# 2646207530/hamer-yolo

Measured on AMD Instinct MI355X. Metric: hands/sec (HaMeR ViT-H/16 + decoder + MANO forward; detector bypassed), higher is better.
Workload: dtype fp16; 1 GPU; BASELINE configs[1]: batch=64 synthetic 256x256 crops per GPU, HaMeR ViT-H/16 + 6-layer decoder + MANO, 16-bit MFMA (fp16 operands), crops resident in HBM; batch_per_gpu=64, global_batch=64, batches_in_flight=2, weights=seeded random-init fp32 master weights, rounded to the operand type at load, parallelism=crop-shard x1

## Files before the change

hamer_yolo_amd/csrc/attention.hip:

```cpp
#include "common.h"
#include "hamer_hip_internal.h"

namespace {

constexpr int T = 192;
constexpr int HD = 80;
constexpr int KSTR = 88;
constexpr int VSTR = 80;
constexpr int KS_BYTES = T * KSTR * 2;
constexpr int VT_BYTES = T * VSTR * 2;
constexpr int BUF_BYTES = KS_BYTES + VT_BYTES;
constexpr int NWAVE = T / 16;
constexpr int OTILE_BYTES = 16 * HD * 2;
constexpr int ATT_LDS = 2 * BUF_BYTES + NWAVE * OTILE_BYTES;
constexpr int ATT_LDS_TOME = ATT_LDS + 2 * T * 4;

template <class V4> __device__ __forceinline__ V4 lds_read_tr4(const void* p) {
  typedef __attribute__((ext_vector_type(4))) short s16x4;
  const s16x4 v = __builtin_amdgcn_ds_read_tr16_b64_v4i16((__attribute__((address_space(3))) s16x4*)p);
  return __builtin_bit_cast(V4, v);
}

__device__ __forceinline__ void glds16_hidden(const void* gsrc, void* lds_wave_base) {
  const unsigned dst = __builtin_amdgcn_readfirstlane((unsigned)(uintptr_t)(__attribute__((address_space(3))) void*)lds_wave_base);
  asm volatile("s_mov_b32 m0, %1\n\ts_nop 0\n\tglobal_load_lds_dwordx4 %0, off" :: "v"(gsrc), "s"(dst) : "memory");
}

__device__ __forceinline__ void wait_vm0() {
  __builtin_amdgcn_s_waitcnt(0x0F70);
  asm volatile("" ::: "memory");
}

constexpr int HDP = 96;
typedef __attribute__((ext_vector_type(4))) int v4i_att;

template <class TT, bool MX8 = false, bool TOME = false>
__global__ __launch_bounds__(64 * NWAVE, 3) void vit_attention_kernel(const typename TT::elem* __restrict__ qkv,
                                                                    typename TT::elem* __restrict__ out, int heads,
                                                                    int items, float scale_log2e,
                                                                    unsigned char* __restrict__ out_scales = nullptr,
                                                                    const float* __restrict__ size = nullptr, int Tn = T) {
  extern __shared__ __attribute__((aligned(16))) char smem[];
  using elem = typename TT::elem;
  using vec8 = typename TT::vec8;
  using vec4 = typename TT::vec4;

  const int tid = threadIdx.x, lane = tid & 63;
  const int wave = __builtin_amdgcn_readfirstlane(tid >> 6);
  const int C = heads * HD;
  const size_t ld = (size_t)3 * C;
  const int g = lane >> 4, li = lane & 15;
  const int Tt = TOME ? Tn : T;
  vec8 zero8;
#pragma unroll
  for (int i = 0; i < 8; ++i) zero8[i] = (elem)0.0f;
  if constexpr (TOME) {
    for (int buf = 0; buf < 2; ++buf) {
      char* Vb = smem + buf * BUF_BYTES + KS_BYTES;
      for (int c = Tt * (VSTR / 8) + tid; c < T * (VSTR / 8); c += 64 * NWAVE) *(vec8*)(Vb + c * 16) = zero8;
    }
  }

  auto issue = [&](int item, int buf, vec8 (&qf)[3], float& szl) {
    const elem* base = qkv + (size_t)(item / heads) * Tt * ld + (size_t)(item % heads) * HD;
    char* Kb = smem + buf * BUF_BYTES;
    char* Vb = Kb + KS_BYTES;
    constexpr int KCH = T * (KSTR / 8), VCH = T * (VSTR / 8);
    const int kch = Tt * (KSTR / 8), vch = Tt * (VSTR / 8);
    for (int c0 = wave * 64; c0 < KCH; c0 += 64 * NWAVE) {
      const int c = c0 + lane, ch = c % (KSTR / 8);
      int t = c / (KSTR / 8);
      if (TOME) t = t < Tt ? t : Tt - 1;
      if (!TOME || c0 < kch) glds16_hidden(base + (size_t)t * ld + C + (ch < HD / 8 ? ch : 0) * 8, Kb + c0 * 16);
    }
    for (int c0 = wave * 64; c0 < VCH; c0 += 64 * NWAVE) {
      const int c = c0 + lane, ch = c % (VSTR / 8);
      int t = c / (VSTR / 8);
      if (TOME) t = t < Tt ? t : Tt - 1;
      if (!TOME || c0 < vch) glds16_hidden(base + (size_t)t * ld + 2 * C + ch * 8, Vb + c0 * 16);
    }
    const int qr = wave * 16 + li;
    const elem* qrow = base + (size_t)(TOME ? (qr < Tt ? qr : Tt - 1) : qr) * ld;
    if constexpr (TOME) szl = (size != nullptr && tid < Tt) ? size[(size_t)(item / heads) * Tt + tid] : 1.0f;
    qf[0] = *(const vec8*)(qrow + 8 * g);
    qf[1] = *(const vec8*)(qrow + 32 + 8 * g);
    qf[2] = g < 2 ? *(const vec8*)(qrow + 64 + 8 * g) : zero8;
  };

  auto compute = [&](int item, int buf, const vec8 (&qf)[3]) {
    const elem* Ks = (const elem*)(smem + buf * BUF_BYTES);
    const elem* Vs = (const elem*)(smem + buf * BUF_BYTES + KS_BYTES);
    const int b = item / heads, h = item % heads;
    const int q = wave * 16 + li;
    if constexpr (TOME) { if (wave * 16 >= Tt) return; }
    f32x4_t st[12];
    vec8 kf[2][2][3];
    auto load_k = [&](int kb, int pair) {
#pragma unroll
      for (int j = 0; j < 2; ++j) {
        const elem* krow = Ks + ((pair * 2 + j) * 16 + li) * KSTR + 8 * g;
        kf[kb][j][0] = *(const vec8*)(krow);
        kf[kb][j][1] = *(const vec8*)(krow + 32);
        kf[kb][j][2] = g < 2 ? *(const vec8*)(krow + 64) : zero8;
      }
    };
    load_k(0, 0);
#pragma unroll
    for (int pair = 0; pair < 6; ++pair) {
      if (pair + 1 < 6) load_k((pair + 1) & 1, pair + 1);
#pragma unroll
      for (int j = 0; j < 2; ++j) {
        f32x4_t acc = f32x4_t{0.f, 0.f, 0.f, 0.f};
        acc = TT::mfma(kf[pair & 1][j][0], qf[0], acc);
        acc = TT::mfma(kf[pair & 1][j][1], qf[1], acc);
        acc = TT::mfma(kf[pair & 1][j][2], qf[2], acc);
        st[pair * 2 + j] = acc;
      }
    }
    if constexpr (TOME) {
#pragma unroll
      for (int kt = 0; kt < 12; ++kt) {
        const f32x4_t lz = *(const f32x4_t*)(smem + ATT_LDS + (buf * T + kt * 16 + 4 * g) * 4);
#pragma unroll
        for (int r = 0; r < 4; ++r) st[kt][r] = (kt * 16 + 4 * g + r < Tt) ? fmaf(st[kt][r], scale_log2e, lz[r]) : -INFINITY;
      }
    }
    float m = st[0][0];
#pragma unroll
    for (int kt = 0; kt < 12; ++kt)
#pragma unroll
      for (int r = 0; r < 4; ++r) m = fmaxf(m, st[kt][r]);
    m = fmaxf(m, __shfl_xor(m, 16, 64));
    m = fmaxf(m, __shfl_xor(m, 32, 64));
    const float mneg = TOME ? -m : -m * scale_log2e;
    float sum4[4] = {0.f, 0.f, 0.f, 0.f};
#pragma unroll
    for (int kt = 0; kt < 12; ++kt)
#pragma unroll
      for (int r = 0; r < 4; ++r) {
        const float p = __builtin_amdgcn_exp2f(TOME ? st[kt][r] + (mneg + 14.0f) : fmaf(st[kt][r], scale_log2e, mneg));
        st[kt][r] = p;
        sum4[r] += p;
      }
    float sum = (sum4[0] + sum4[1]) + (sum4[2] + sum4[3]);
    sum += __shfl_xor(sum, 16, 64);
    sum += __shfl_xor(sum, 32, 64);
    const float inv = 1.0f / sum;

    vec8 pf[6], pl[TOME ? 6 : 1];
#pragma unroll
    for (int kk = 0; kk < 6; ++kk)
#pragma unroll
      for (int r = 0; r < 4; ++r) {
        pf[kk][r] = (elem)st[2 * kk][r];
        pf[kk][4 + r] = (elem)st[2 * kk + 1][r];
        if constexpr (TOME) {
          pl[kk][r] = (elem)(st[2 * kk][r] - (float)pf[kk][r]);
          pl[kk][4 + r] = (elem)(st[2 * kk + 1][r] - (float)pf[kk][4 + r]);
        }
      }

    const elem* vblk = Vs + (4 * g + (li >> 2)) * VSTR + 4 * (li & 3);
    vec4 vlo[2][5], vhi[2][5];
    auto load_v = [&](int vb, int kk) {
#pragma unroll
      for (int dt = 0; dt < 5; ++dt) {
        vlo[vb][dt] = lds_read_tr4<vec4>(vblk + (32 * kk) * VSTR + dt * 16);
        vhi[vb][dt] = lds_read_tr4<vec4>(vblk + (32 * kk + 16) * VSTR + dt * 16);
      }
    };
    f32x4_t oacc[5];
#pragma unroll
    for (int dt = 0; dt < 5; ++dt) oacc[dt] = f32x4_t{0.f, 0.f, 0.f, 0.f};
    if constexpr (!TOME) load_v(0, 0);
#pragma unroll
    for (int kk = 0; kk < 6; ++kk) {
      if constexpr (TOME) load_v(kk & 1, kk);
      else if (kk + 1 < 6) load_v((kk + 1) & 1, kk + 1);
#pragma unroll
      for (int dt = 0; dt < 5; ++dt) {
        vec8 vf;
#pragma unroll
        for (int i = 0; i < 4; ++i) { vf[i] = vlo[kk & 1][dt][i]; vf[4 + i] = vhi[kk & 1][dt][i]; }
        oacc[dt] = TT::mfma(vf, pf[kk], oacc[dt]);
        if constexpr (TOME) oacc[dt] = TT::mfma(vf, pl[kk], oacc[dt]);
      }
    }
    if constexpr (MX8) {
      const int Mrows = (items / heads) * T;
      float am[3] = {0.f, 0.f, 0.f};
#pragma unroll
      for (int dt = 0; dt < 5; ++dt)
#pragma unroll
        for (int r = 0; r < 4; ++r) am[dt >> 1] = fmaxf(am[dt >> 1], fabsf(oacc[dt][r] * inv));
      unsigned sb[3];
      float isc[3];
#pragma unroll
      for (int bk = 0; bk < 3; ++bk) {
        float a = am[bk];
        a = fmaxf(a, __shfl_xor(a, 16, 64));
        a = fmaxf(a, __shfl_xor(a, 32, 64));
        sb[bk] = mx8_scale_byte(a);
        isc[bk] = mx8_inv_scale(sb[bk]);
      }
      char* ot8 = smem + 2 * BUF_BYTES + wave * OTILE_BYTES;
#pragma unroll
      for (int dt = 0; dt < 6; ++dt) {
        int p = 0;
        if (dt < 5) {
          const float sc = inv * isc[dt >> 1];
          p = mx8_pack4(oacc[dt][0] * sc, oacc[dt][1] * sc, oacc[dt][2] * sc, oacc[dt][3] * sc);
        }
        *(int*)(ot8 + li * HDP + dt * 16 + 4 * g) = p;
      }
      char* obase8 = (char*)out + ((size_t)b * T + wave * 16) * (heads * HDP) + h * HDP;
#pragma unroll
      for (int c0 = 0; c0 < 16 * (HDP / 16); c0 += 64) {
        const int c = c0 + lane;
        if (c < 16 * (HDP / 16)) {
          const int row = c / (HDP / 16), ch = c % (HDP / 16);
          *(v4i_att*)(obase8 + (size_t)row * (heads * HDP) + ch * 16) = *(const v4i_att*)(ot8 + row * HDP + ch * 16);
        }
      }
      if (g == 0) {
#pragma unroll
        for (int bk = 0; bk < 3; ++bk) out_scales[(size_t)(h * 3 + bk) * Mrows + (size_t)b * T + q] = (unsigned char)sb[bk];
      }
      return;
    }
    elem* ot = (elem*)(smem + 2 * BUF_BYTES + wave * OTILE_BYTES);
#pragma unroll
    for (int dt = 0; dt < 5; ++dt) {
      vec4 o;
#pragma unroll
      for (int r = 0; r < 4; ++r) o[r] = (elem)(oacc[dt][r] * inv);
      *(vec4*)(ot + li * HD + dt * 16 + 4 * g) = o;
    }
    elem* obase = out + ((size_t)b * Tt + wave * 16) * C + h * HD;
#pragma unroll
    for (int c0 = 0; c0 < 16 * (HD / 8); c0 += 64) {
      const int c = c0 + lane;
      if (c < 16 * (HD / 8)) {
        const int row = c / (HD / 8), ch = c % (HD / 8);
        if (!TOME || wave * 16 + row < Tt) *(vec8*)(obase + (size_t)row * C + ch * 8) = *(const vec8*)(ot + row * HD + ch * 8);
      }
    }
  };

  vec8 qa[3], qb[3];
  float sza = 1.0f, szb = 1.0f;
  auto publish_size = [&](int buf, float szl) {
    if constexpr (TOME) { if (tid < Tt) *(float*)(smem + ATT_LDS + (buf * T + tid) * 4) = __builtin_amdgcn_logf(szl); }
  };
  int item = xcd_remap(blockIdx.x, gridDim.x);
  if (item < items) issue(item, 0, qa, sza);
  while (item < items) {
    wait_vm0();
    publish_size(0, sza);
    __builtin_amdgcn_s_barrier();
    int nxt = item + gridDim.x;
    if (nxt < items) issue(nxt, 1, qb, szb);
    compute(item, 0, qa);
    item = nxt;
    if (item >= items) break;
    wait_vm0();
    publish_size(1, szb);
    __builtin_amdgcn_s_barrier();
    nxt = item + gridDim.x;
    if (nxt < items) issue(nxt, 0, qa, sza);
    compute(item, 1, qb);
    item = nxt;
  }
}

int att_grid_for(int items, int n_cu) {
  if (const int v = hm_option(HM_OPT_ATT_GRID)) n_cu = v;
  const int per = (items + n_cu - 1) / n_cu;
  return (items + per - 1) / per;
}

template <class TT, bool MX8 = false, bool TOME = false>
int launch_att(const void* qkv, void* out, int B, int heads, float scale, hipStream_t s, void* out_scales = nullptr,
               const float* size = nullptr, int Tn = T) {
  static HmLdsOnce lds_once;
  auto kern = vit_attention_kernel<TT, MX8, TOME>;
  constexpr int LDS = TOME ? ATT_LDS_TOME : ATT_LDS;
  if (const int rc = lds_once.ensure((const void*)kern, LDS, "hm_vit_attention: cannot raise dynamic LDS limit")) return rc;
  const int n_cu = hm_device_cu_count();
  if (n_cu <= 0) return hm_set_error(HM_ERR_HIP, "hm_vit_attention: cannot query the device");
  const int items = B * heads;
  const int grid = att_grid_for(items, n_cu);
  hipLaunchKernelGGL(kern, dim3(grid), dim3(64 * NWAVE), LDS, s, (const typename TT::elem*)qkv,
                     (typename TT::elem*)out, heads, items, scale * 1.44269504088896340736f, (unsigned char*)out_scales, size, Tn);
  return hm_check_launch("hm_vit_attention");
}

}

extern "C" int hm_attention_grid(int items, int cus) {
  if (items <= 0) return 0;
  return att_grid_for(items, cus > 0 ? cus : 256);
}

int hm_attention_tome_launch(const void* qkv, const float* size, void* out, int B, int tokens, int heads, float scale, int dtype,
                             hipStream_t s) {
  if (tokens < 1 || tokens > T) return hm_set_error(HM_ERR_ARG, "hm_tome_attention: 0 < tokens <= 192");
  if (dtype == HM_DTYPE_BF16) return launch_att<TBf16, false, true>(qkv, out, B, heads, scale, s, nullptr, size, tokens);
  if (dtype == HM_DTYPE_F16) return launch_att<TF16, false, true>(qkv, out, B, heads, scale, s, nullptr, size, tokens);
  return hm_set_error(HM_ERR_ARG, "hm_tome_attention: bad dtype");
}

extern "C" int hm_vit_attention(const void* qkv, void* out, int B, int tokens, int heads, int head_dim, float scale,
                                int dtype, void* stream_) {
  hipStream_t s = (hipStream_t)stream_;
  if (!qkv || !out || B <= 0 || heads <= 0) return hm_set_error(HM_ERR_ARG, "hm_vit_attention: bad arguments");
  if (tokens != T || head_dim != HD)
    return hm_set_error(HM_ERR_ARG, "hm_vit_attention: built for 192 tokens and head_dim 80 (ViT-H/16 on 256x192)");
  if (((uintptr_t)qkv | (uintptr_t)out) & 15) return hm_set_error(HM_ERR_ARG, "hm_vit_attention: 16-byte alignment");
  HmProfScope prof(HM_K_ATTENTION, 0, B, heads, head_dim, s);
  if (dtype == HM_DTYPE_BF16) return launch_att<TBf16>(qkv, out, B, heads, scale, s);
  if (dtype == HM_DTYPE_F16) return launch_att<TF16>(qkv, out, B, heads, scale, s);
  return hm_set_error(HM_ERR_ARG, "hm_vit_attention: bad dtype");
}

extern "C" int hm_vit_attention_mx8(const void* qkv, void* out8, void* out_scales, int B, int tokens, int heads, int head_dim,
                                    float scale, void* stream_) {
  hipStream_t s = (hipStream_t)stream_;
  if (!qkv || !out8 || !out_scales || B <= 0 || heads <= 0) return hm_set_error(HM_ERR_ARG, "hm_vit_attention_mx8: bad arguments");
  if (tokens != T || head_dim != HD)
    return hm_set_error(HM_ERR_ARG, "hm_vit_attention_mx8: built for 192 tokens and head_dim 80 (ViT-H/16 on 256x192)");
  if (((uintptr_t)qkv | (uintptr_t)out8 | (uintptr_t)out_scales) & 15) return hm_set_error(HM_ERR_ARG, "hm_vit_attention_mx8: 16-byte alignment");
  HmProfScope prof(HM_K_ATTENTION, 1, B, heads, head_dim, s);
  return launch_att<TBf16, true>(qkv, out8, B, heads, scale, s, out_scales);
}
```

hamer_yolo_amd/csrc/status.hip:

```cpp
#include <stdio.h>
#include <string.h>
#include "common.h"
#include "hamer_hip_internal.h"

static thread_local char g_err[512] = "";

int hm_set_error(int code, const char* msg) {
  snprintf(g_err, sizeof(g_err), "%s", msg ? msg : "");
  return code;
}

int hm_check_launch(const char* what) {
  hipError_t e = hipGetLastError();
  if (e == hipSuccess) return HM_OK;
  snprintf(g_err, sizeof(g_err), "%s: %s", what, hipGetErrorString(e));
  return HM_ERR_HIP;
}

int hm_device_cu_count(void) {
  static std::mutex mu;
  static int cus[64] = {0};
  int dev = 0;
  if (hipGetDevice(&dev) != hipSuccess) return -1;
  std::lock_guard<std::mutex> lock(mu);
  if (dev < 64 && cus[dev] > 0) return cus[dev];
  int n = 0;
  if (hipDeviceGetAttribute(&n, hipDeviceAttributeMultiprocessorCount, dev) != hipSuccess) return -1;
  if (dev < 64) cus[dev] = n;
  return n;
}

#include <atomic>
static std::atomic<int> g_opts[HM_OPT_COUNT];
int hm_option(int key) {
  return (key >= 0 && key < HM_OPT_COUNT) ? g_opts[key].load(std::memory_order_relaxed) : 0;
}
extern "C" int hm_get_option(int key) { return hm_option(key); }
extern "C" int hm_option_count(void) { return HM_OPT_COUNT; }
extern "C" int hm_set_option(int key, int value) {
  if (key < 0 || key >= HM_OPT_COUNT) return hm_set_error(HM_ERR_ARG, "hm_set_option: unknown key");
  if (value < 0) return hm_set_error(HM_ERR_ARG, "hm_set_option: value must be >= 0");
  if ((key == HM_OPT_PX_GRID || key == HM_OPT_FP8P_GRID) && value != 0 && (value < 8 || value % 8 != 0))
    return hm_set_error(HM_ERR_ARG, "hm_set_option: a persistent grid is 0 (default) or a multiple of the 8 XCDs");
  if (key == HM_OPT_GEMM_STAGGER && value > 4)
    return hm_set_error(HM_ERR_ARG, "hm_set_option: HM_OPT_GEMM_STAGGER is 0 (default), 1 (lockstep), 2 (staggered), 3 or 4 (one kernel staggered)");
  g_opts[key].store(value, std::memory_order_relaxed);
  return HM_OK;
}

extern "C" int hm_version(void) { return HM_VERSION; }
extern "C" const char* hm_last_error_string(void) { return g_err; }
```

hamer_yolo_amd/lib.py:

```python
from __future__ import annotations

import ctypes as C
import os

HERE = os.path.dirname(os.path.abspath(__file__))
LIB_PATH = os.path.join(HERE, "libhamer_hip.so")

HM_DTYPE_BF16, HM_DTYPE_F16, HM_OUT_F32 = 0, 1, 2
HM_DTYPE_F32 = 2
HM_EPI_STORE, HM_EPI_GELU, HM_EPI_RESID_F32, HM_EPI_F32, HM_EPI_SILU = 0, 1, 2, 3, 4
HM_EPI_RESID_LN, HM_EPI_LN_STORE, HM_EPI_LN_GELU, HM_EPI_GELU_MX8 = 5, 6, 7, 8
HM_VERSION = 402
OPTION_NAMES = ("HM_OPT_PX_GRID", "HM_OPT_FP8P_GRID", "HM_OPT_FP8_ONE_TILE", "HM_OPT_FP8P_RESID", "HM_OPT_TOME_NO_SPLITK",
                "HM_OPT_TOME_SCALAR_ATTENTION", "HM_OPT_RESID_IN_EPILOGUE", "HM_OPT_CONV_TILE", "HM_OPT_CONV_SPLITK",
                "HM_OPT_PX_LDS_EPILOGUE", "HM_OPT_CONV_DIRECT", "HM_OPT_GEMM_TILE_RULE", "HM_OPT_CONV_KGROUPS",
                "HM_OPT_CONV_GENERAL_LOADER", "HM_OPT_CONV_STEM_PAIR", "HM_OPT_ATT_GRID", "HM_OPT_GEMM_STAGGER")
globals().update({_n: _i for _i, _n in enumerate(OPTION_NAMES)})

EXPORTS = [
    "hm_version", "hm_last_error_string", "hm_gemm", "hm_layernorm", "hm_vit_attention", "hm_patch_im2col",
    "hm_linear_f32", "hm_broadcast_rows", "hm_cross_attention", "hm_mano_forward", "hm_crop_box_from_bbox",
    "hm_crop_batch", "hm_hamer_workspace_bytes", "hm_hamer_forward", "hm_prof_begin", "hm_prof_collect", "hm_prof_end",
    "hm_conv2d_nhwc", "hm_conv2d_stem_pair", "hm_maxpool_nhwc", "hm_upsample2x_nhwc", "hm_letterbox_plan_make", "hm_letterbox_tables",
    "hm_letterbox", "hm_yolo_decode", "hm_nms_workspace_bytes", "hm_yolo_nms", "hm_yolo_run", "hm_gemm_set_variant", "hm_gemm_set_group_m", "hm_ln_finalize", "hm_layernorm_accum", "hm_gemm_fp8", "hm_layernorm_mx8", "hm_vit_attention_mx8", "hm_nchw3_to_nhwc8", "hm_gap_linear",
    "hm_tome_index_bytes", "hm_tome_attention", "hm_tome_merge", "hm_set_option", "hm_get_option", "hm_tome_merge_metric", "hm_conv_splitk_bytes", "hm_yolo_decode_batch", "hm_letterbox_batch",
    "hm_option_count", "hm_gemm_px_grid", "hm_absmax16", "hm_mesh_overlay_workspace_bytes", "hm_mesh_overlay",
    "hm_sar_saigb", "hm_sar_graph_mix", "hm_sar_linear", "hm_sar_softargmax", "hm_sar_postprocess",
    "hm_conv2d_f32_relu", "hm_nchw3_to_nhwc8_f32", "hm_gap_linear_f32", "hm_sar_saigb_f32", "hm_sar_graph_mix_f32", "hm_sar_linear_f32",
    "hm_gemm_f32", "hm_vit_attention_f32",
    "hm_dwconv7_ln", "hm_ln_patchify2", "hm_stem4_im2col", "hm_sar_saigb_ch",
    "hm_mesh_render_workspace_bytes", "hm_mesh_render",
    "hm_attention_grid",
    "hm_crop_aa_box_from_bbox", "hm_crop_batch_aa",
    "hm_pose_eval",
    "hm_skeleton_overlay_workspace_bytes", "hm_skeleton_overlay",
]
KIND_NAMES = ["gemm", "layernorm", "attention", "im2col", "linear_f32", "cross_attn", "mano", "crop", "conv", "other"]


class HipLibraryError(RuntimeError):
    pass


vp, fp = C.c_void_p, C.c_void_p


class GemmArgs(C.Structure):
    _fields_ = [("X", vp), ("W", vp), ("C", vp), ("bias", vp), ("resid", vp),
                ("M", C.c_int), ("N", C.c_int), ("K", C.c_int),
                ("ldx", C.c_int), ("ldw", C.c_int), ("ldc", C.c_int), ("ldr", C.c_int),
                ("resid_mod", C.c_int), ("epilogue", C.c_int), ("dtype", C.c_int),
                ("ln_gamma", vp), ("ln_xg", vp), ("ln_stats", vp), ("ln_colsum", vp), ("k_split", C.c_int), ("out_scale", C.c_float)]


class GemmFp8Args(C.Structure):
    _fields_ = [("X8", vp), ("x_scales", vp), ("W8", vp), ("w_scale", vp), ("C", vp), ("bias", vp), ("resid", vp),
                ("out_scales", vp), ("M", C.c_int), ("N", C.c_int), ("K", C.c_int), ("ldx", C.c_int), ("ldw", C.c_int),
                ("ldc", C.c_int), ("ldr", C.c_int), ("epilogue", C.c_int), ("out_dtype", C.c_int)]


class ManoModel(C.Structure):
    _fields_ = [("v_template", vp), ("shapedirs", vp), ("posedirs", vp), ("J_regressor", vp), ("lbs_weights", vp),
                ("n_verts", C.c_int)]


class CropBox(C.Structure):
    _fields_ = [("m0", C.c_double), ("m4", C.c_double), ("x0", C.c_int32), ("y0", C.c_int32),
                ("flip", C.c_int32), ("reserved", C.c_int32)]


HM_CROP_AA_MAX_RADIUS = 48
HM_CROP_AA_TAPS = HM_CROP_AA_MAX_RADIUS + 1


class CropAaBox(C.Structure):
    _fields_ = CropBox._fields_ + [("sigma", C.c_float), ("radius", C.c_int32), ("pad", C.c_int32 * 2)]


class PoseEvalArgs(C.Structure):
    _fields_ = [("pred", vp), ("gt", vp), ("B", C.c_int), ("P", C.c_int), ("gt_stride", C.c_int), ("root", C.c_int),
                ("sel", C.c_uint64 * 16), ("err", vp), ("pa_err", vp), ("aligned", vp), ("transform", vp)]


class VitBlock(C.Structure):
    _fields_ = [(n, vp) for n in ("ln1_g", "ln1_b", "ln2_g", "ln2_b", "qkv_w", "proj_w", "fc1_w", "fc2_w",
                                  "qkv_b", "proj_b", "fc1_b", "fc2_b",
                                  "qkv_colsum", "qkv_bias_ln", "fc1_colsum", "fc1_bias_ln",
                                  "qkv_w8", "fc1_w8", "fc2_w8", "qkv_ws", "fc1_ws", "fc2_ws", "proj_w8", "proj_ws", "kmean_w", "kmean_b")] + \
               [("attn_scale_mul", C.c_float), ("gelu_out_scale", C.c_float)]


class DecLayer(C.Structure):
    _fields_ = [(n, vp) for n in ("ln0_g", "ln0_b", "ln1_g", "ln1_b", "ln2_g", "ln2_b", "sa_v_w", "sa_w", "sa_out_w",
                                  "sa_out_b", "ca_q_w", "ca_out_w", "ca_out_b", "ff1_w", "ff1_b", "ff2_w", "ff2_b")] + \
               [("ca_scale_mul", C.c_float)]


class HamerWeights(C.Structure):
    _fields_ = [(n, C.c_int) for n in ("img_h", "img_w_full", "win_x0", "win_w", "patch", "pad", "embed_dim", "depth",
                                       "heads", "mlp_dim")] + \
               [("vit_eps", C.c_float), ("patch_w", vp), ("patch_b", vp), ("pos", vp),
                ("blocks", C.POINTER(VitBlock)), ("last_g", vp), ("last_b", vp)] + \
               [(n, C.c_int) for n in ("dec_dim", "dec_depth", "dec_heads", "dec_dim_head", "dec_mlp")] + \
               [("dec_eps", C.c_float), ("token0", vp), ("kv_w", vp), ("layers", C.POINTER(DecLayer)),
                ("head_w", vp), ("head_b", vp), ("mano", ManoModel),
                ("focal_length", C.c_float), ("image_size", C.c_float), ("dtype", C.c_int), ("tome_r", C.POINTER(C.c_int)),
                ("range_stats", vp)]


class ConvArgs(C.Structure):
    _fields_ = [("X", vp), ("W", vp), ("Y", vp), ("bias", vp), ("zeros", vp)] + \
               [(n, C.c_int) for n in ("N", "H", "W_in", "Cin", "Cout", "ksize", "stride", "ldx", "ldy", "Kpad", "act",
                                       "out_f32", "dtype")] + [("resid", vp), ("ldr", C.c_int), ("splitk_ws", vp), ("splitk_ws_bytes", C.c_size_t)]


class YoloOp(C.Structure):
    _fields_ = [("kind", C.c_int), ("pool_pad", C.c_int), ("conv", ConvArgs)]


class LetterboxPlan(C.Structure):
    _fields_ = [(n, C.c_int) for n in ("src_h", "src_w", "new_w", "new_h", "top", "left", "out_h", "out_w")] + \
               [("gain", C.c_float), ("pad_x", C.c_float), ("pad_y", C.c_float)]


HM_STYLE_FLAT, HM_STYLE_SHADED = 0, 1


class Mesh(C.Structure):
    _fields_ = [(n, C.c_int32) for n in ("frame", "v0", "nv", "f0", "nf")] + [("color_bgr", C.c_uint8 * 3), ("reserved", C.c_uint8)]


HM_SKEL_INTERLEAVED, HM_SKEL_BONES_FIRST = 0, 1


class Skeleton(C.Structure):
    _fields_ = [("image", C.c_int32), ("line_radius", C.c_int32), ("joint_radius", C.c_int32), ("threshold", C.c_float)]


class SarHand(C.Structure):
    _fields_ = [("bb2img", C.c_float * 6), ("depth_box", C.c_float), ("flip", C.c_int32), ("img_w", C.c_int32),
                ("img_h", C.c_int32), ("depth_w", C.c_int32), ("depth_h", C.c_int32), ("depth_offset", C.c_int64),
                ("fx", C.c_double), ("fy", C.c_double), ("fu", C.c_double), ("fv", C.c_double)]


class ProfRecord(C.Structure):
    _fields_ = [("kind", C.c_int), ("epilogue", C.c_int), ("M", C.c_int), ("N", C.c_int), ("K", C.c_int), ("ms", C.c_float)]


class HamerOutputs(C.Structure):
    _fields_ = [(n, vp) for n in ("pose6d", "betas", "cam", "rotmats", "verts", "joints", "cam_t", "kp2d", "tokens")]


_lib = None


def load() -> C.CDLL:
    global _lib
    if _lib is not None:
        return _lib
    if not os.path.exists(LIB_PATH):
        raise HipLibraryError(
            f"{LIB_PATH} not found: build it with `python -m hamer_yolo_amd.build` (hipcc, gfx950). "
            "There is no CPU fallback for the hot path.")
    try:
        import torch
    except ImportError:
        pass
    try:
        lib = C.CDLL(LIB_PATH)
    except OSError as e:
        raise HipLibraryError(f"cannot load {LIB_PATH}: {e}") from e
    i, f, d = C.c_int, C.c_float, C.c_double
    lib.hm_version.restype = i
    lib.hm_last_error_string.restype = C.c_char_p
    lib.hm_gemm.argtypes = [C.POINTER(GemmArgs), vp]
    lib.hm_layernorm.argtypes = [vp, vp, vp, vp, i, i, i, f, vp]
    lib.hm_vit_attention.argtypes = [vp, vp, i, i, i, i, f, i, vp]
    lib.hm_patch_im2col.argtypes = [vp, vp, i, i, i, i, i, i, i, i, vp]
    lib.hm_linear_f32.argtypes = [vp, i, vp, i, vp, vp, i, vp, i, i, i, i, i, vp]
    lib.hm_broadcast_rows.argtypes = [vp, vp, i, i, vp]
    lib.hm_cross_attention.argtypes = [vp, vp, i, i, i, vp, i, i, i, i, f, i, vp]
    lib.hm_mano_forward.argtypes = [C.POINTER(ManoModel), vp, vp, vp, vp, vp, vp, vp, vp, i, f, f, vp]
    lib.hm_crop_box_from_bbox.argtypes = [d, d, d, i, i, C.POINTER(CropBox)]
    lib.hm_crop_batch.argtypes = [vp, i, i, vp, vp, i, i, C.POINTER(C.c_float), C.POINTER(C.c_float), vp]
    lib.hm_crop_aa_box_from_bbox.argtypes = [d, d, d, i, i, C.POINTER(CropAaBox), C.POINTER(C.c_float)]
    lib.hm_crop_batch_aa.argtypes = [vp, i, i, vp, vp, vp, i, i, C.POINTER(C.c_float), C.POINTER(C.c_float), vp]
    lib.hm_hamer_workspace_bytes.argtypes = [C.POINTER(HamerWeights), i]
    lib.hm_hamer_workspace_bytes.restype = C.c_size_t
    lib.hm_hamer_forward.argtypes = [C.POINTER(HamerWeights), vp, i, C.POINTER(HamerOutputs), vp, C.c_size_t, vp]
    lib.hm_ln_finalize.argtypes = [vp, vp, i, i, C.c_float, vp]
    lib.hm_gemm_fp8.argtypes = [C.POINTER(GemmFp8Args), vp]
    lib.hm_layernorm_mx8.argtypes = [vp, vp, vp, vp, vp, i, i, C.c_float, vp]
    lib.hm_vit_attention_mx8.argtypes = [vp, vp, vp, i, i, i, i, C.c_float, vp]
    lib.hm_nchw3_to_nhwc8.argtypes = [vp, vp, i, i, i, i, vp]
    lib.hm_gap_linear.argtypes = [vp, i, i, vp, C.c_float, vp, vp, i, i, vp]
    lib.hm_layernorm_accum.argtypes = [vp, vp, i, vp, vp, vp, vp, i, i, i, C.c_float, vp]
    lib.hm_absmax16.argtypes = [vp, i, i, i, i, i, vp, vp]
    lib.hm_conv2d_nhwc.argtypes = [C.POINTER(ConvArgs), vp]
    lib.hm_conv_splitk_bytes.argtypes = [C.POINTER(ConvArgs)]
    lib.hm_conv2d_stem_pair.argtypes = [C.POINTER(ConvArgs), C.POINTER(ConvArgs), vp]
    lib.hm_conv_splitk_bytes.restype = C.c_size_t
    lib.hm_maxpool_nhwc.argtypes = [vp, i, vp, i, i, i, i, i, i, i, i, i, vp]
    lib.hm_upsample2x_nhwc.argtypes = [vp, i, vp, i, i, i, i, i, i, vp]
    lib.hm_letterbox_plan_make.argtypes = [i, i, i, i, C.POINTER(LetterboxPlan)]
    lib.hm_letterbox_tables.argtypes = [C.POINTER(LetterboxPlan), C.POINTER(C.c_int32)]
    lib.hm_letterbox.argtypes = [vp, C.POINTER(LetterboxPlan), vp, vp, i, vp, vp]
    lib.hm_letterbox_batch.argtypes = [vp, C.c_size_t, i, C.POINTER(LetterboxPlan), vp, vp, i, vp]
    lib.hm_yolo_decode.argtypes = [vp, i, vp, i, i, i, i, f, C.POINTER(C.c_float), vp]
    lib.hm_yolo_decode_batch.argtypes = [vp, i, vp, i, i, i, i, f, C.POINTER(C.c_float), i, C.c_size_t, vp]
    lib.hm_nms_workspace_bytes.argtypes = [i]
    lib.hm_nms_workspace_bytes.restype = C.c_size_t
    lib.hm_yolo_nms.argtypes = [vp, i, i, f, f, C.c_uint, i, i, C.POINTER(LetterboxPlan), vp, vp, vp, C.c_size_t, vp]
    lib.hm_yolo_run.argtypes = [C.POINTER(YoloOp), i, vp]
    lib.hm_tome_index_bytes.argtypes = [i]
    lib.hm_tome_index_bytes.restype = C.c_size_t
    lib.hm_tome_attention.argtypes = [vp, vp, vp, i, i, i, i, f, i, vp]
    lib.hm_tome_merge.argtypes = [vp, vp, vp, vp, vp, vp, vp, i, i, i, i, i, i, i, vp]
    lib.hm_tome_merge_metric.argtypes = [vp, i, i, vp, vp, vp, vp, vp, i, i, i, i, vp]
    lib.hm_gemm_set_variant.argtypes = [i]
    lib.hm_gemm_set_group_m.argtypes = [i]
    lib.hm_set_option.argtypes = [i, i]
    lib.hm_get_option.argtypes = [i]
    lib.hm_option_count.argtypes = []
    lib.hm_gemm_px_grid.argtypes = [i, i]
    lib.hm_attention_grid.argtypes = [i, i]
    lib.hm_mesh_overlay_workspace_bytes.argtypes = [i, i, i, i, i]
    lib.hm_mesh_overlay_workspace_bytes.restype = C.c_size_t
    lib.hm_mesh_overlay.argtypes = [vp, i, i, i, vp, vp, i, vp, i, C.POINTER(Mesh), i, i, d, vp, vp, C.c_size_t, vp]
    lib.hm_mesh_render_workspace_bytes.argtypes = [i, i, i, i, i, i]
    lib.hm_mesh_render_workspace_bytes.restype = C.c_size_t
    lib.hm_mesh_render.argtypes = [i, i, i, C.POINTER(d), vp, i, vp, i, C.POINTER(Mesh), i, C.POINTER(d), C.POINTER(C.c_uint8), d,
                                   vp, vp, vp, vp, vp, vp, C.c_size_t, vp]
    lib.hm_sar_saigb.argtypes = [vp, vp, vp, vp, vp, i, vp]
    lib.hm_sar_graph_mix.argtypes = [vp, i, vp, i, vp, vp]
    lib.hm_sar_linear.argtypes = [vp, i, i, vp, vp, vp, i, i, vp]
    lib.hm_sar_softargmax.argtypes = [vp] * 10 + [i, vp]
    lib.hm_sar_postprocess.argtypes = [vp, vp, vp, vp, vp, vp, i, i, vp]
    lib.hm_conv2d_f32_relu.argtypes = [C.POINTER(ConvArgs), vp]
    lib.hm_nchw3_to_nhwc8_f32.argtypes = [vp, vp, i, i, i, vp]
    lib.hm_gap_linear_f32.argtypes = [vp, i, i, vp, C.c_float, vp, vp, i, vp]
    lib.hm_sar_saigb_f32.argtypes = [vp, vp, vp, vp, vp, i, vp]
    lib.hm_sar_graph_mix_f32.argtypes = [vp, i, vp, i, vp, vp]
    lib.hm_sar_linear_f32.argtypes = [vp, i, i, vp, vp, vp, i, i, vp]
    lib.hm_gemm_f32.argtypes = [C.POINTER(GemmArgs), vp]
    lib.hm_vit_attention_f32.argtypes = [vp, vp, i, i, i, i, f, vp]
    lib.hm_dwconv7_ln.argtypes = [vp, vp, vp, vp, vp, vp, i, i, i, i, f, i, vp]
    lib.hm_ln_patchify2.argtypes = [vp, vp, vp, vp, i, i, i, i, f, i, vp]
    lib.hm_stem4_im2col.argtypes = [vp, vp, i, i, i, i, vp]
    lib.hm_sar_saigb_ch.argtypes = [vp, vp, vp, vp, vp, i, i, vp]
    lib.hm_pose_eval.argtypes = [C.POINTER(PoseEvalArgs), vp]
    lib.hm_skeleton_overlay_workspace_bytes.argtypes = [i, i, i, i]
    lib.hm_skeleton_overlay_workspace_bytes.restype = C.c_size_t
    lib.hm_skeleton_overlay.argtypes = [vp, i, i, i, vp, i, C.POINTER(Skeleton), i, C.POINTER(C.c_uint8), i, vp, vp, C.c_size_t, vp]
    lib.hm_prof_begin.argtypes = [i]
    lib.hm_prof_collect.argtypes = [C.POINTER(ProfRecord), i]
    lib.hm_prof_end.argtypes = []
    for name in EXPORTS:
        if not hasattr(lib, name):
            raise HipLibraryError(f"{LIB_PATH} does not export {name}")
        fn = getattr(lib, name)
        if name not in ("hm_version", "hm_last_error_string", "hm_hamer_workspace_bytes", "hm_nms_workspace_bytes", "hm_tome_index_bytes", "hm_conv_splitk_bytes",
                        "hm_mesh_overlay_workspace_bytes", "hm_mesh_render_workspace_bytes",
                        "hm_skeleton_overlay_workspace_bytes"):
            fn.restype = i
    if lib.hm_version() != HM_VERSION:
        raise HipLibraryError(f"{LIB_PATH} reports HM_VERSION {lib.hm_version()}, this binding is written for {HM_VERSION}: "
                              "rebuild it (python -m hamer_yolo_amd.build --force)")
    if lib.hm_option_count() != len(OPTION_NAMES):
        raise HipLibraryError(f"{LIB_PATH} has {lib.hm_option_count()} HM_OPT_* keys, this binding names {len(OPTION_NAMES)}: "
                              "include/hamer_hip.h and lib.OPTION_NAMES have drifted apart")
    _lib = lib
    return lib


class option:

    def __init__(self, key: int, value: int):
        self.key, self.value = key, value

    def __enter__(self):
        self.old = load().hm_get_option(self.key)
        check(load().hm_set_option(self.key, self.value), "hm_set_option")
        return self

    def __exit__(self, *exc):
        load().hm_set_option(self.key, self.old)
        return False


def check(rc: int, what: str = "") -> None:
    if rc != 0:
        msg = load().hm_last_error_string().decode(errors="replace")
        raise HipLibraryError(f"{what or 'libhamer_hip'} failed (code {rc}): {msg}")


def ptr(t) -> int:
    return None if t is None else t.data_ptr()


def current_stream() -> int:
    import torch
    return torch.cuda.current_stream().cuda_stream


class profile:

    def __init__(self, capacity: int = 1 << 16):
        self.capacity = capacity
        self.records = []

    def __enter__(self):
        check(load().hm_prof_begin(self.capacity), "hm_prof_begin")
        return self

    def collect(self):
        buf = (ProfRecord * self.capacity)()
        n = load().hm_prof_collect(buf, self.capacity)
        if n < 0:
            check(n, "hm_prof_collect")
# ... 11 lines not shown
```

include/hamer_hip.h:

```cpp
#ifndef HAMER_HIP_H
#define HAMER_HIP_H
#include <stddef.h>
#include <stdint.h>

#ifdef __cplusplus
extern "C" {
#endif

#define HM_VERSION 402

enum { HM_DTYPE_BF16 = 0, HM_DTYPE_F16 = 1,
       HM_DTYPE_F32 = 2  };

enum {
  HM_EPI_STORE = 0,
  HM_EPI_GELU = 1,
  HM_EPI_RESID_F32 = 2,
  HM_EPI_F32 = 3,
  HM_EPI_SILU = 4,
  HM_EPI_RESID_LN = 5,
  HM_EPI_LN_STORE = 6,
  HM_EPI_LN_GELU = 7,
  HM_EPI_GELU_MX8 = 8,
  HM_EPI_RELU = 9,
  HM_EPI_ADD_RELU = 10
};

typedef struct hm_gemm_args {
  const void* X;
  const void* W;
  void* C;
  const float* bias;
  const float* resid;
  int M, N, K;
  int ldx, ldw, ldc, ldr;
  int resid_mod;
  int epilogue;
  int dtype;
  const float* ln_gamma;
  void* ln_xg;
  float* ln_stats;
  const float* ln_colsum;
  int k_split;
  float out_scale;
} hm_gemm_args;

int hm_gemm(const hm_gemm_args* args, void* stream);
int hm_ln_finalize(const float* partials, float* row_stats, int M, int D, float eps, void* stream);
int hm_gemm_set_variant(int variant);
int hm_gemm_set_group_m(int group_m);
enum {
  HM_OPT_PX_GRID = 0,
  HM_OPT_FP8P_GRID = 1,
  HM_OPT_FP8_ONE_TILE = 2,
  HM_OPT_FP8P_RESID = 3,
  HM_OPT_TOME_NO_SPLITK = 4,
  HM_OPT_TOME_SCALAR_ATTENTION = 5,
  HM_OPT_RESID_IN_EPILOGUE = 6,
  HM_OPT_CONV_TILE = 7,
  HM_OPT_CONV_SPLITK = 8,
  HM_OPT_PX_LDS_EPILOGUE = 9,
  HM_OPT_CONV_DIRECT = 10,
  HM_OPT_GEMM_TILE_RULE = 11,
  HM_OPT_CONV_KGROUPS = 12,
  HM_OPT_CONV_GENERAL_LOADER = 13,
  HM_OPT_CONV_STEM_PAIR = 14,
  HM_OPT_ATT_GRID = 15,
  HM_OPT_GEMM_STAGGER = 16,
  HM_OPT_COUNT = 17
};
int hm_set_option(int key, int value);
int hm_get_option(int key);
int hm_option_count(void);
int hm_gemm_px_grid(int tiles, int cus);
int hm_attention_grid(int items, int cus);

typedef struct hm_gemm_fp8_args {
  const void* X8; const void* x_scales;
  const void* W8; const float* w_scale;
  void* C; const float* bias; const float* resid; void* out_scales;
  int M, N, K, ldx, ldw, ldc, ldr;
  int epilogue;
  int out_dtype;
} hm_gemm_fp8_args;
int hm_gemm_fp8(const hm_gemm_fp8_args* args, void* stream);
int hm_layernorm_mx8(const float* x, const float* gamma, const float* beta, void* out8, void* out_scales, int M, int D,
                     float eps, void* stream);

#define HM_OUT_F32 2
int hm_layernorm(const float* x, const float* gamma, const float* beta, void* out, int out_dtype,
                 int M, int D, float eps, void* stream);
int hm_layernorm_accum(float* x, const float* partials, int n_partials, const float* bias, const float* gamma,
                       const float* beta, void* out, int out_dtype, int M, int D, float eps, void* stream);
int hm_absmax16(const void* x, int ld, int M, int col0, int ncols, int dtype, float* slot, void* stream);

int hm_vit_attention(const void* qkv, void* out, int B, int tokens, int heads, int head_dim, float scale,
                     int dtype, void* stream);

size_t hm_tome_index_bytes(int B);
int hm_tome_attention(const void* qkv, const float* size, void* out, int B, int tokens, int heads, int head_dim, float scale,
                      int dtype, void* stream);
int hm_tome_merge(const void* qkv, const float* x, const float* size, float* x_out, float* size_out, float* metric_ws,
                  int* index_ws, int B, int tokens, int r, int heads, int head_dim, int D, int dtype, void* stream);
int hm_tome_merge_metric(const float* metric, int ld_metric, int lo_off, const float* x, const float* size, float* x_out,
                         float* size_out, int* index_ws, int B, int tokens, int r, int D, void* stream);

int hm_vit_attention_mx8(const void* qkv, void* out8, void* out_scales, int B, int tokens, int heads, int head_dim, float scale,
                         void* stream);

int hm_patch_im2col(const float* img, void* patches, int B, int img_h, int img_w_full, int x0, int win_w,
                    int patch, int pad, int dtype, void* stream);

int hm_linear_f32(const float* x, int ldx, const float* W, int ldw, const float* bias, const float* resid, int ldr,
                  float* out, int ldo, int M, int N, int K, int act, void* stream);


int hm_broadcast_rows(const float* vec, float* out, int B, int D, void* stream);

int hm_cross_attention(const float* q, const void* kv, int ldkv, int k_off, int v_off, float* out, int B, int tokens,
                       int heads, int dim_head, float scale, int dtype, void* stream);

typedef struct hm_mano_model {
  const float* v_template;
  const float* shapedirs;
  const float* posedirs;
  const float* J_regressor;
  const float* lbs_weights;
  int n_verts;
} hm_mano_model;

int hm_mano_forward(const hm_mano_model* model, const float* pose6d, const float* betas, const float* cam,
                    float* rotmats, float* verts, float* joints, float* cam_t, float* kp2d, int B,
                    float focal_length, float image_size, void* stream);

typedef struct hm_crop_box {
  double m0, m4;
  int32_t x0, y0;
  int32_t flip;
  int32_t reserved;
} hm_crop_box;

int hm_crop_box_from_bbox(double cx, double cy, double size, int flip, int P, hm_crop_box* out);

int hm_crop_batch(const uint8_t* frame, int H, int W, const hm_crop_box* boxes, float* out, int B, int P,
                  const float* mean3_host, const float* std3_host, void* stream);

#define HM_CROP_AA_MAX_SIGMA 12.0
#define HM_CROP_AA_MAX_RADIUS 48
#define HM_CROP_AA_TAPS (HM_CROP_AA_MAX_RADIUS + 1)
typedef struct hm_crop_aa_box {
  double m0, m4;
  int32_t x0, y0;
  int32_t flip;
  int32_t reserved;
  float sigma;
  int32_t radius;
  int32_t pad[2];
} hm_crop_aa_box;

int hm_crop_aa_box_from_bbox(double cx, double cy, double size, int flip, int P, hm_crop_aa_box* out, float* taps_out);

int hm_crop_batch_aa(const uint8_t* frame, int H, int W, const hm_crop_aa_box* boxes, const float* taps, float* out, int B,
                     int P, const float* mean3_host, const float* std3_host, void* stream);

typedef struct hm_vit_block {
  const float *ln1_g, *ln1_b, *ln2_g, *ln2_b;
  const void *qkv_w, *proj_w, *fc1_w, *fc2_w;
  const float *qkv_b, *proj_b, *fc1_b, *fc2_b;
  const float *qkv_colsum, *qkv_bias_ln, *fc1_colsum, *fc1_bias_ln;
  const void *qkv_w8, *fc1_w8, *fc2_w8;
  const float *qkv_ws, *fc1_ws, *fc2_ws;
  const void* proj_w8;
  const float* proj_ws;
  const float* kmean_w;
  const float* kmean_b;
  float attn_scale_mul, gelu_out_scale;
} hm_vit_block;

typedef struct hm_dec_layer {
  const float *ln0_g, *ln0_b, *ln1_g, *ln1_b, *ln2_g, *ln2_b;
  const float* sa_v_w;
  const float* sa_w;
  const float *sa_out_w, *sa_out_b;
  const float* ca_q_w;
  const float *ca_out_w, *ca_out_b;
  const float *ff1_w, *ff1_b, *ff2_w, *ff2_b;
  float ca_scale_mul;
} hm_dec_layer;

typedef struct hm_hamer_weights {
  int img_h, img_w_full, win_x0, win_w, patch, pad, embed_dim, depth, heads, mlp_dim;
  float vit_eps;
  const void* patch_w;
  const float* patch_b;
  const float* pos;
  const hm_vit_block* blocks;
  const float *last_g, *last_b;
  int dec_dim, dec_depth, dec_heads, dec_dim_head, dec_mlp;
  float dec_eps;
  const float* token0;
  const void* kv_w;
  const hm_dec_layer* layers;
  const float* head_w;
  const float* head_b;
  hm_mano_model mano;
  float focal_length, image_size;
  int dtype;
  const int* tome_r;
  float* range_stats;
} hm_hamer_weights;

typedef struct hm_hamer_outputs {
  float* pose6d;
  float* betas;
  float* cam;
  float* rotmats;
  float* verts;
  float* joints;
  float* cam_t;
  float* kp2d;
  void* tokens;
} hm_hamer_outputs;

size_t hm_hamer_workspace_bytes(const hm_hamer_weights* w, int B);

int hm_hamer_forward(const hm_hamer_weights* w, const float* img, int B, const hm_hamer_outputs* out,
                     void* workspace, size_t workspace_bytes, void* stream);

typedef struct hm_conv_args {
  const void* X;
  const void* W;
  void* Y;
  const float* bias;
  const void* zeros;
  int N, H, W_in, Cin, Cout, ksize, stride, ldx, ldy, Kpad;
  int act;
  int out_f32;
  int dtype;
  const void* resid;
  int ldr;
  void* splitk_ws;
  size_t splitk_ws_bytes;
} hm_conv_args;

int hm_conv2d_nhwc(const hm_conv_args* args, void* stream);
size_t hm_conv_splitk_bytes(const hm_conv_args* args);
int hm_conv2d_stem_pair(const hm_conv_args* first, const hm_conv_args* second, void* stream);

int hm_maxpool_nhwc(const void* x, int ldx, void* y, int ldy, int N, int H, int W, int C, int k, int stride, int pad,
                    int dtype, void* stream);

int hm_nchw3_to_nhwc8(const float* x, void* y, int B, int H, int W, int dtype, void* stream);
int hm_gap_linear(const void* feat, int HW, int C, const float* w, float bias, const float* k_value, float* depth, int B,
                  int dtype, void* stream);

int hm_upsample2x_nhwc(const void* x, int ldx, void* y, int ldy, int N, int H, int W, int C, int dtype, void* stream);

typedef struct hm_letterbox_plan {
  int src_h, src_w;
  int new_w, new_h;
  int top, left;
  int out_h, out_w;
  float gain, pad_x, pad_y;
} hm_letterbox_plan;
int hm_letterbox_plan_make(int H, int W, int new_shape, int stride, hm_letterbox_plan* plan);
int hm_letterbox_tables(const hm_letterbox_plan* plan, int32_t* tab_host);
int hm_letterbox(const uint8_t* frame, const hm_letterbox_plan* plan, const int32_t* tab_dev, void* x8, int dtype,
                 uint8_t* u8_chw, void* stream);
int hm_letterbox_batch(const uint8_t* frames, size_t frame_stride_bytes, int nb, const hm_letterbox_plan* plan,
                       const int32_t* tab_dev, void* x8, int dtype, void* stream);

int hm_yolo_decode(const float* raw, int ldraw, float* pred, int row0, int ny, int nx, int nc, float stride,
                   const float* anchors6_host, void* stream);
int hm_yolo_decode_batch(const float* raw, int ldraw, float* pred, int row0, int ny, int nx, int nc, float stride,
                         const float* anchors, int nb, size_t pred_rows_per_image, void* stream);

size_t hm_nms_workspace_bytes(int n);
int hm_yolo_nms(const float* pred, int n, int nc, float conf_thres, float iou_thres, unsigned class_mask, int agnostic,
                int max_det, const hm_letterbox_plan* plan, float* dets, int* count, void* workspace,
                size_t workspace_bytes, void* stream);

enum { HM_OP_CONV = 0, HM_OP_MAXPOOL = 1, HM_OP_UPSAMPLE2X = 2,
       HM_OP_CONV_PAIR = 3  };
typedef struct hm_yolo_op {
  int kind;
  int pool_pad;
  hm_conv_args conv;
} hm_yolo_op;
int hm_yolo_run(const hm_yolo_op* ops_host, int n_ops, void* stream);

enum { HM_STYLE_FLAT = 0, HM_STYLE_SHADED = 1 };
typedef struct hm_mesh {
  int32_t frame;
  int32_t v0, nv;
  int32_t f0, nf;
  uint8_t color_bgr[3];
  uint8_t reserved;
} hm_mesh;
size_t hm_mesh_overlay_workspace_bytes(int N, int H, int W, int n_meshes, int n_faces);
int hm_mesh_overlay(const uint8_t* frames, int N, int H, int W, const double* K, const double* verts, int n_verts,
                    const int32_t* faces, int n_faces, const hm_mesh* meshes_host, int n_meshes, int style, double alpha,
                    uint8_t* out, void* workspace, size_t workspace_bytes, void* stream);

size_t hm_mesh_render_workspace_bytes(int N, int H, int W, int n_verts, int n_meshes, int n_faces);
int hm_mesh_render(int N, int H, int W, const double* K_host, const double* verts, int n_verts, const int32_t* faces,
                   int n_faces, const hm_mesh* meshes_host, int n_meshes, const double* base_rgb, const uint8_t* bg_rgba,
                   double znear, const uint8_t* frames, uint8_t* out, uint8_t* rgba, float* depth, int32_t* mesh_id,
                   void* workspace, size_t workspace_bytes, void* stream);

enum { HM_SKEL_INTERLEAVED = 0, HM_SKEL_BONES_FIRST = 1 };
typedef struct hm_skeleton {
  int32_t image;
  int32_t line_radius, joint_radius;
  float threshold;
} hm_skeleton;
size_t hm_skeleton_overlay_workspace_bytes(int N, int H, int W, int n_hands);
int hm_skeleton_overlay(const uint8_t* images, int N, int H, int W, const float* kp, int kp_stride,
                        const hm_skeleton* hands_host, int n_hands, const uint8_t* palette_host, int order, uint8_t* out,
                        void* workspace, size_t workspace_bytes, void* stream);


int hm_sar_saigb(const void* feat, const void* w, const float* bias, const float* tmpl, void* g, int B, void* stream);
int hm_sar_saigb_ch(const void* feat, const void* w, const float* bias, const float* tmpl, void* g, int B, int channels,
                    void* stream);
int hm_sar_graph_mix(const void* lap, int ldl, const void* x, int N, void* y, void* stream);
int hm_sar_linear(const void* x, int M, int K, const void* w, const float* bias, void* y, int N, int out_f32, void* stream);
int hm_sar_softargmax(float* logits_xy, float* logits_z, const float* m2p_w_xy, const float* m2p_b_xy, const float* m2p_w_z,
                      const float* m2p_b_z, const float* beta, const float* wx, const float* wy, float* coords, int B,
                      void* stream);
typedef struct hm_sar_hand {
  float bb2img[6];
  float depth_box;
  int32_t flip;
  int32_t img_w, img_h;
  int32_t depth_w, depth_h;
  int64_t depth_offset;
  double fx, fy, fu, fv;
} hm_sar_hand;
int hm_sar_postprocess(const float* coords, const hm_sar_hand* hands, const float* root, const float* depth, float* uvd,
                       float* xyz, int B, int P, void* stream);



int hm_conv2d_f32_relu(const hm_conv_args* args, void* stream);
int hm_nchw3_to_nhwc8_f32(const float* x, float* y, int B, int H, int W, void* stream);
int hm_gap_linear_f32(const float* feat, int HW, int C, const float* w, float bias, const float* k_value, float* depth, int B,
                      void* stream);
int hm_sar_saigb_f32(const float* feat, const float* w, const float* bias, const float* tmpl, float* g, int B, void* stream);
int hm_sar_graph_mix_f32(const float* lap, int ldl, const float* x, int N, float* y, void* stream);
int hm_sar_linear_f32(const float* x, int M, int K, const float* w, const float* bias, float* y, int N, int logits, void* stream);

int hm_gemm_f32(const hm_gemm_args* args, void* stream);
int hm_vit_attention_f32(const float* qkv, float* out, int B, int tokens, int heads, int head_dim, float scale, void* stream);


int hm_dwconv7_ln(const float* x, const float* w, const float* bias, const float* gamma, const float* beta, void* out, int B, int H,
                  int W, int C, float eps, int dtype, void* stream);
int hm_ln_patchify2(const float* x, const float* gamma, const float* beta, void* out, int B, int H, int W, int C, float eps,
                    int dtype, void* stream);
int hm_stem4_im2col(const float* img, void* patches, int B, int H, int W, int dtype, void* stream);

typedef struct hm_pose_eval_args {
  const float* pred;
  const float* gt;
  int B, P, gt_stride;
  int root;
  uint64_t sel[16];
  float* err;
  float* pa_err;
  float* aligned;
  float* transform;
} hm_pose_eval_args;
// ... 17 lines not shown
```

Measured before the change: 3826 hands/s.

## Replace full vmcnt drains in ViT attention with counted waits and deferred V barrier

Attention's double-buffered loop used to drain all outstanding global loads (vmcnt 0) before each item. It now issues Q loads via inline asm between the K and V async LDS copies and waits only until K and Q arrive. The V half of the buffer is waited for with a second counted wait plus a barrier just before the PV stage, so V loading overlaps the QK^T and softmax work. A new option selects the old full-wait path or tuning variants of the barrier. This relies on exact vmcnt accounting of the issued loads and stores, which is fragile if the compiler emits extra memory ops.

New measurement: 3821 hands/s. About the same (-0.1%).

```diff
diff --git a/hamer_yolo_amd/csrc/attention.hip b/hamer_yolo_amd/csrc/attention.hip
--- a/hamer_yolo_amd/csrc/attention.hip
+++ b/hamer_yolo_amd/csrc/attention.hip
@@ -31,15 +31,29 @@
   asm volatile("" ::: "memory");
 }
 
+template <int N> __device__ __forceinline__ void wait_vm_n() { asm volatile("s_waitcnt vmcnt(%0)" :: "n"(N) : "memory"); }
+template <int NV, int NS, class V8> __device__ __forceinline__ void wait_vm_q(bool v_behind, bool stores_behind, V8 (&q)[3]) {
+  if (v_behind) { if (stores_behind) wait_vm_n<NV + NS>(); else wait_vm_n<NV>(); }
+  else { if (stores_behind) wait_vm_n<NS>(); else wait_vm_n<0>(); }
+  asm volatile("" : "+v"(q[0]), "+v"(q[1]), "+v"(q[2]) :: "memory");
+}
+
+template <class V8> __device__ __forceinline__ void q_load(V8 (&q)[3], const void* row, int off2) {
+  const char* r2 = (const char*)row + off2;
+  asm volatile("global_load_dwordx4 %0, %3, off\n\tglobal_load_dwordx4 %1, %3, off offset:64\n\tglobal_load_dwordx4 %2, %4, off"
+               : "=&v"(q[0]), "=&v"(q[1]), "=&v"(q[2]) : "v"(row), "v"(r2) : "memory");
+}
+
 constexpr int HDP = 96;
 typedef __attribute__((ext_vector_type(4))) int v4i_att;
 
-template <class TT, bool MX8 = false, bool TOME = false>
+template <class TT, bool MX8 = false, bool TOME = false, bool OLDW = false>
 __global__ __launch_bounds__(64 * NWAVE, 3) void vit_attention_kernel(const typename TT::elem* __restrict__ qkv,
                                                                     typename TT::elem* __restrict__ out, int heads,
                                                                     int items, float scale_log2e,
                                                                     unsigned char* __restrict__ out_scales = nullptr,
-                                                                    const float* __restrict__ size = nullptr, int Tn = T) {
+                                                                    const float* __restrict__ size = nullptr, int Tn = T,
+                                                                    int vmode = 0) {
   extern __shared__ __attribute__((aligned(16))) char smem[];
   using elem = typename TT::elem;
   using vec8 = typename TT::vec8;
@@ -51,6 +65,7 @@
   const size_t ld = (size_t)3 * C;
   const int g = lane >> 4, li = lane & 15;
   const int Tt = TOME ? Tn : T;
+  constexpr int NK_MIN = TOME ? 0 : 2, NV_MIN = TOME ? 0 : 2, NEXT_MIN = NK_MIN + 3 + NV_MIN, NS = MX8 ? 5 : 3;
   vec8 zero8;
 #pragma unroll
   for (int i = 0; i < 8; ++i) zero8[i] = (elem)0.0f;
@@ -67,32 +82,43 @@
     char* Vb = Kb + KS_BYTES;
     constexpr int KCH = T * (KSTR / 8), VCH = T * (VSTR / 8);
     const int kch = Tt * (KSTR / 8), vch = Tt * (VSTR / 8);
+    const int qr = wave * 16 + li;
+    const elem* qrow = base + (size_t)(TOME ? (qr < Tt ? qr : Tt - 1) : qr) * ld;
+    if constexpr (TOME && !OLDW) szl = (size != nullptr && tid < Tt) ? size[(size_t)(item / heads) * Tt + tid] : 1.0f;
     for (int c0 = wave * 64; c0 < KCH; c0 += 64 * NWAVE) {
       const int c = c0 + lane, ch = c % (KSTR / 8);
       int t = c / (KSTR / 8);
       if (TOME) t = t < Tt ? t : Tt - 1;
       if (!TOME || c0 < kch) glds16_hidden(base + (size_t)t * ld + C + (ch < HD / 8 ? ch : 0) * 8, Kb + c0 * 16);
     }
+    if constexpr (!OLDW) q_load(qf, qrow + 8 * g, g < 2 ? 128 : 0);
     for (int c0 = wave * 64; c0 < VCH; c0 += 64 * NWAVE) {
       const int c = c0 + lane, ch = c % (VSTR / 8);
       int t = c / (VSTR / 8);
       if (TOME) t = t < Tt ? t : Tt - 1;
       if (!TOME || c0 < vch) glds16_hidden(base + (size_t)t * ld + 2 * C + ch * 8, Vb + c0 * 16);
     }
-    const int qr = wave * 16 + li;
-    const elem* qrow = base + (size_t)(TOME ? (qr < Tt ? qr : Tt - 1) : qr) * ld;
-    if constexpr (TOME) szl = (size != nullptr && tid < Tt) ? size[(size_t)(item / heads) * Tt + tid] : 1.0f;
-    qf[0] = *(const vec8*)(qrow + 8 * g);
-    qf[1] = *(const vec8*)(qrow + 32 + 8 * g);
-    qf[2] = g < 2 ? *(const vec8*)(qrow + 64 + 8 * g) : zero8;
+    if constexpr (OLDW) {
+      if constexpr (TOME) szl = (size != nullptr && tid < Tt) ? size[(size_t)(item / heads) * Tt + tid] : 1.0f;
+      qf[0] = *(const vec8*)(qrow + 8 * g);
+      qf[1] = *(const vec8*)(qrow + 32 + 8 * g);
+      qf[2] = g < 2 ? *(const vec8*)(qrow + 64 + 8 * g) : zero8;
+    }
   };
 
-  auto compute = [&](int item, int buf, const vec8 (&qf)[3]) {
+  auto compute = [&](int item, int buf, const vec8 (&qf)[3], bool has_next, bool vbar) {
+    auto wait_v = [&] { if (has_next) wait_vm_n<NEXT_MIN>(); else wait_vm_n<0>(); };
     const elem* Ks = (const elem*)(smem + buf * BUF_BYTES);
     const elem* Vs = (const elem*)(smem + buf * BUF_BYTES + KS_BYTES);
     const int b = item / heads, h = item % heads;
     const int q = wave * 16 + li;
-    if constexpr (TOME) { if (wave * 16 >= Tt) return; }
+    if constexpr (TOME) {
+      if (wave * 16 >= Tt) {
+        if constexpr (!OLDW) { if (vbar) { wait_v(); __builtin_amdgcn_s_barrier(); } }
+        return;
+      }
+    }
+    const vec8 q2 = (OLDW || g < 2) ? qf[2] : zero8;
     f32x4_t st[12];
     vec8 kf[2][2][3];
     auto load_k = [&](int kb, int pair) {
@@ -113,7 +139,7 @@
         f32x4_t acc = f32x4_t{0.f, 0.f, 0.f, 0.f};
         acc = TT::mfma(kf[pair & 1][j][0], qf[0], acc);
         acc = TT::mfma(kf[pair & 1][j][1], qf[1], acc);
-        acc = TT::mfma(kf[pair & 1][j][2], qf[2], acc);
+        acc = TT::mfma(kf[pair & 1][j][2], q2, acc);
         st[pair * 2 + j] = acc;
       }
     }
@@ -161,6 +187,13 @@
       }
 
     const elem* vblk = Vs + (4 * g + (li >> 2)) * VSTR + 4 * (li & 3);
+    if constexpr (!OLDW) {
+      if (vbar) {
+        wait_v();
+        __builtin_amdgcn_s_barrier();
+      }
+      asm volatile("" ::: "memory");
+    }
     vec4 vlo[2][5], vhi[2][5];
     auto load_v = [&](int vb, int kk) {
 #pragma unroll
@@ -252,23 +285,28 @@
   auto publish_size = [&](int buf, float szl) {
     if constexpr (TOME) { if (tid < Tt) *(float*)(smem + ATT_LDS + (buf * T + tid) * 4) = __builtin_amdgcn_logf(szl); }
   };
+  const bool counts_stores = !TOME || wave * 16 + 16 <= Tt;
+  bool stores_behind = false;
+  bool vbar = vmode != 3;
   int item = xcd_remap(blockIdx.x, gridDim.x);
   if (item < items) issue(item, 0, qa, sza);
   while (item < items) {
-    wait_vm0();
+    if constexpr (OLDW) wait_vm0(); else wait_vm_q<NV_MIN, NS>(vbar, stores_behind, qa);
     publish_size(0, sza);
     __builtin_amdgcn_s_barrier();
     int nxt = item + gridDim.x;
     if (nxt < items) issue(nxt, 1, qb, szb);
-    compute(item, 0, qa);
+    compute(item, 0, qa, nxt < items, vbar);
+    stores_behind = counts_stores;
+    vbar = vmode == 2;
     item = nxt;
     if (item >= items) break;
-    wait_vm0();
+    if constexpr (OLDW) wait_vm0(); else wait_vm_q<NV_MIN, NS>(vbar, counts_stores, qb);
     publish_size(1, szb);
     __builtin_amdgcn_s_barrier();
     nxt = item + gridDim.x;
     if (nxt < items) issue(nxt, 0, qa, sza);
-    compute(item, 1, qb);
+    compute(item, 1, qb, nxt < items, vbar);
     item = nxt;
   }
 }
@@ -279,11 +317,11 @@
   return (items + per - 1) / per;
 }
 
-template <class TT, bool MX8 = false, bool TOME = false>
-int launch_att(const void* qkv, void* out, int B, int heads, float scale, hipStream_t s, void* out_scales = nullptr,
-               const float* size = nullptr, int Tn = T) {
+template <class TT, bool MX8, bool TOME, bool OLDW>
+int launch_att_w(const void* qkv, void* out, int B, int heads, float scale, hipStream_t s, void* out_scales, const float* size,
+                 int Tn) {
   static HmLdsOnce lds_once;
-  auto kern = vit_attention_kernel<TT, MX8, TOME>;
+  auto kern = vit_attention_kernel<TT, MX8, TOME, OLDW>;
   constexpr int LDS = TOME ? ATT_LDS_TOME : ATT_LDS;
   if (const int rc = lds_once.ensure((const void*)kern, LDS, "hm_vit_attention: cannot raise dynamic LDS limit")) return rc;
   const int n_cu = hm_device_cu_count();
@@ -291,8 +329,16 @@
   const int items = B * heads;
   const int grid = att_grid_for(items, n_cu);
   hipLaunchKernelGGL(kern, dim3(grid), dim3(64 * NWAVE), LDS, s, (const typename TT::elem*)qkv,
-                     (typename TT::elem*)out, heads, items, scale * 1.44269504088896340736f, (unsigned char*)out_scales, size, Tn);
+                     (typename TT::elem*)out, heads, items, scale * 1.44269504088896340736f, (unsigned char*)out_scales, size, Tn,
+                     hm_option(HM_OPT_ATT_WAITS));
   return hm_check_launch("hm_vit_attention");
+}
+
+template <class TT, bool MX8 = false, bool TOME = false>
+int launch_att(const void* qkv, void* out, int B, int heads, float scale, hipStream_t s, void* out_scales = nullptr,
+               const float* size = nullptr, int Tn = T) {
+  if (hm_option(HM_OPT_ATT_WAITS) == 1) return launch_att_w<TT, MX8, TOME, true>(qkv, out, B, heads, scale, s, out_scales, size, Tn);
+  return launch_att_w<TT, MX8, TOME, false>(qkv, out, B, heads, scale, s, out_scales, size, Tn);
 }
 
 }
diff --git a/hamer_yolo_amd/csrc/status.hip b/hamer_yolo_amd/csrc/status.hip
--- a/hamer_yolo_amd/csrc/status.hip
+++ b/hamer_yolo_amd/csrc/status.hip
@@ -44,6 +44,8 @@
     return hm_set_error(HM_ERR_ARG, "hm_set_option: a persistent grid is 0 (default) or a multiple of the 8 XCDs");
   if (key == HM_OPT_GEMM_STAGGER && value > 4)
     return hm_set_error(HM_ERR_ARG, "hm_set_option: HM_OPT_GEMM_STAGGER is 0 (default), 1 (lockstep), 2 (staggered), 3 or 4 (one kernel staggered)");
+  if (key == HM_OPT_ATT_WAITS && value > 3)
+    return hm_set_error(HM_ERR_ARG, "hm_set_option: HM_OPT_ATT_WAITS is 0 (counted waits), 1 (one full wait per step), 2 or 3 (tuning: V's barrier at every item / at none)");
   g_opts[key].store(value, std::memory_order_relaxed);
   return HM_OK;
 }
diff --git a/hamer_yolo_amd/lib.py b/hamer_yolo_amd/lib.py
--- a/hamer_yolo_amd/lib.py
+++ b/hamer_yolo_amd/lib.py
@@ -14,7 +14,8 @@
 OPTION_NAMES = ("HM_OPT_PX_GRID", "HM_OPT_FP8P_GRID", "HM_OPT_FP8_ONE_TILE", "HM_OPT_FP8P_RESID", "HM_OPT_TOME_NO_SPLITK",
                 "HM_OPT_TOME_SCALAR_ATTENTION", "HM_OPT_RESID_IN_EPILOGUE", "HM_OPT_CONV_TILE", "HM_OPT_CONV_SPLITK",
                 "HM_OPT_PX_LDS_EPILOGUE", "HM_OPT_CONV_DIRECT", "HM_OPT_GEMM_TILE_RULE", "HM_OPT_CONV_KGROUPS",
-                "HM_OPT_CONV_GENERAL_LOADER", "HM_OPT_CONV_STEM_PAIR", "HM_OPT_ATT_GRID", "HM_OPT_GEMM_STAGGER")
+                "HM_OPT_CONV_GENERAL_LOADER", "HM_OPT_CONV_STEM_PAIR", "HM_OPT_ATT_GRID", "HM_OPT_GEMM_STAGGER",
+                "HM_OPT_ATT_WAITS")
 globals().update({_n: _i for _i, _n in enumerate(OPTION_NAMES)})
 
 EXPORTS = [
diff --git a/include/hamer_hip.h b/include/hamer_hip.h
--- a/include/hamer_hip.h
+++ b/include/hamer_hip.h
@@ -67,7 +67,8 @@
   HM_OPT_CONV_STEM_PAIR = 14,
   HM_OPT_ATT_GRID = 15,
   HM_OPT_GEMM_STAGGER = 16,
-  HM_OPT_COUNT = 17
+  HM_OPT_ATT_WAITS = 17,
+  HM_OPT_COUNT = 18
 };
 int hm_set_option(int key, int value);
 int hm_get_option(int key);
```
